# lc700x/desktop2stereo

Measured on AMD Instinct MI355X. Metric: stereo frames/sec @1080p DepthAnything-v2-ViT-B, higher is better.
Workload: dtype bf16; 1 GPU; DepthAnything-v2-vitb bf16, 1920x1080 uint8 RGB noise frames, batch 1 per GPU, Depth Resolution 518 (model input 294x518), Full-SBS uint8 output 3840x1080, pred; parallelism=frame-sharded dp1, no data-path collective (each rank generates its own frames)

## Files before the change

### desktop2stereo_amd/csrc/engine.hip

```cpp
#include <map>
#include <string>
#include <vector>
#include <cmath>
#include <cstring>

#include "gemm.h"
#include "linear_site.h"
#include "vit_ops.h"

using namespace d2s;

namespace {

struct HostT { std::vector<float> data; std::vector<int64_t> shape; };

struct PackedW {
    void* w = nullptr;
    float* bias = nullptr;
    int N = 0, K = 0, Kpad = 0;
};

struct Layer {
    float *ln1g, *ln1b, *ln2g, *ln2b, *ls1, *ls2;
    PackedW qkv, proj, fc1, fc2;
// ... 193 lines not shown
    auto c1 = [&](float x) { return ((A + 2.f) * x - (A + 3.f)) * x * x + 1.f; };
    auto c2 = [&](float x) { return ((A * x - 5.f * A) * x + 8.f * A) * x - 4.f * A; };
    c[0] = c2(t + 1.f); c[1] = c1(t); c[2] = c1(1.f - t); c[3] = c2(2.f - t);
}

void interp_pos(const float* pos, int grid, int D, int gh, int gw, std::vector<float>& out, double offset = 0.0) {
    out.assign((size_t)(1 + gh * gw) * D, 0.f);
    std::memcpy(out.data(), pos, D * sizeof(float));
    if (gh == grid && gw == grid) { std::memcpy(out.data() + D, pos + D, (size_t)grid * grid * D * sizeof(float)); return; }
    float sy = (float)grid / (float)gh, sx = (float)grid / (float)gw;
    if (offset != 0.0) {
        sy = (float)(1.0 / (((double)gh + offset) / (double)grid)); sx = (float)(1.0 / (((double)gw + offset) / (double)grid));
    }
    for (int oy = 0; oy < gh; ++oy) {
        float fy = sy * ((float)oy + 0.5f) - 0.5f;
        float iyf = floorf(fy);
        float cy[4]; cubic_coeffs(fy - iyf, cy);
        int iy = (int)iyf;
        for (int ox = 0; ox < gw; ++ox) {
            float fx = sx * ((float)ox + 0.5f) - 0.5f;
            float ixf = floorf(fx);
            float cx[4]; cubic_coeffs(fx - ixf, cx);
            int ix = (int)ixf;
            float* o = out.data() + (size_t)(1 + oy * gw + ox) * D;
            for (int d = 0; d < D; ++d) {
                float acc = 0.f;
                for (int a = 0; a < 4; ++a) {
                    int yy = std::min(std::max(iy - 1 + a, 0), grid - 1);
                    float row = 0.f;
                    for (int b = 0; b < 4; ++b) {
                        int xx = std::min(std::max(ix - 1 + b, 0), grid - 1);
                        row += pos[(size_t)(1 + yy * grid + xx) * D + d] * cx[b];
                    }
                    acc += row * cy[a];
                }
                o[d] = acc;
            }
        }
    }
}

GemmA plainA(const void* p, long lda) { GemmA a = {}; a.ptr = p; a.mode = A_PLAIN; a.lda = lda; return a; }
GemmA splitA(const void* p, long lda, bool split) { GemmA a = plainA(p, lda); a.bx3 = split ? 1 : 0; return a; }
GemmA convA(const void* p, int Hi, int Wi, int C, int Ho, int Wo, int stride, int relu) {
    GemmA a = {}; a.ptr = p; a.mode = A_CONV3; a.Hi = Hi; a.Wi = Wi; a.C = C; a.Ho = Ho; a.Wo = Wo; a.stride = stride; a.relu = relu; return a;
}

int gemm(d2s_engine* e, const GemmA& a, const PackedW& w, int M, const GemmEpi& ep, hipStream_t st) {
    int Kl = w.K % (e->prec == D2S_PREC_BF16 ? 8 : 4) ? w.Kpad : w.K;
    GemmEpi ep2 = ep;
    if (ep.map == MAP_ROWS) {
        ep2.part = (e->side && st == e->side) ? e->splitk_ws_side : e->splitk_ws;
        ep2.part_elems = e->splitk_elems;
    }
    PROF(a.mode == A_CONV3 ? PC_CONV : PC_GEMM, 2.0 * M * w.N * w.K, 0, launch_gemm(e->wprec, 0, a, w.w, M, w.N, Kl, w.Kpad, ep2, st));
    return D2S_OK;
}

int gemm8(d2s_engine* e, const GemmA& a, const PackedW& w, int M, const GemmEpi& ep, hipStream_t st) {
    PROF(PC_GEMM, 2.0 * M * w.N * w.K, 0, launch_gemm(D2S_PREC_FP8_OPERANDS, 0, a, w.w, M, w.N, w.K, w.Kpad, ep, st));
    return D2S_OK;
}

int conv3(d2s_engine* e, const void* in, int B, int Hi, int Wi, int C, int stride, int relu_in, const PackedW& w,
          void* out, int act, const void* res1, const void* res2, hipStream_t st) {
    int Ho = (Hi + 2 - 3) / stride + 1, Wo = (Wi + 2 - 3) / stride + 1;
    GemmA a = convA(in, Hi, Wi, C, Ho, Wo, stride, relu_in);
    GemmEpi ep = rowsE(out, OUT_T, w.N, w.bias);
    ep.act = act; ep.res1 = res1; ep.res2 = res2;
    return gemm(e, a, w, B * Ho * Wo, ep, st);
}

void window_rows(const d2s_engine::TSlot& sl, bool fold, void* ring, AttnRow& attn, CacheRow& store) {
    const bool in_attn = fold && sl.filled;
    attn = AttnRow{ring, (int16_t)sl.head, (int16_t)(sl.filled ? 32 : 1), in_attn ? sl.head : -1};
    store = CacheRow{ring, sl.filled ? sl.head : 0, sl.filled ? (in_attn ? 0 : 1) : 31};
}

int run_temporal(d2s_engine* e, int m, const void* x, void* out, int B, hipStream_t st, const void* add = nullptr) {
    d2s_engine::TMod& t = e->tm[m];
    const int C = t.C, S = B * t.sites, prec = e->prec;
    const int* ids = e->row_ids;
    const bool fold = e->tm_fold;
    int slots = 0;
    auto producer = [&](GemmEpi& ep) { if (fold) epi_ln_producer(ep, e->tm_a, e->tm_stats, &slots); };
    auto consumer = [&](GemmEpi& ep, const float* csum) { epi_ln_consumer(ep, e->tm_stats, slots, csum, 1e-5f, C); };
    void* gn_out = fold ? e->tm_out : e->tm_a;
    PROF(PC_ELT, 0, 0, launch_groupnorm(prec, x, t.gn_g, t.gn_b, gn_out, t.sites, C, 32, 1e-6f, st, B));
    {
        GemmEpi ep = rowsE(e->tm_hs, OUT_F32, C, t.proj_in.bias);
        producer(ep);
        RC(gemm(e, plainA(gn_out, C), t.proj_in, S, ep, st));
    }
    for (int a = 0; a < 2; ++a) {
        const bool folded = fold && slots >= 1 && slots <= 16;
        if (!folded) PROF(PC_LN, 0, 0, launch_layernorm(prec, e->tm_hs, t.ln_g[a], t.ln_b[a], e->tm_a, S, C, 1e-5f, 0, 0, 0, st));
        {
            GemmEpi ep = rowsE(e->tm_kv, OUT_T, 3 * C, folded ? t.kvq_ln[a].bias : nullptr);
            if (folded) consumer(ep, t.csum_kvq[a]);
            RC(gemm(e, plainA(e->tm_a, C), folded ? t.kvq_ln[a] : t.kvq[a], S, ep, st));
        }
        AttnRows attn = {};
        CacheRows store = {};
        double win_rows = 0;
        bool store_due = false;
        for (int r = 0; r < B; ++r) {
// ... 745 lines not shown
```

### desktop2stereo_amd/csrc/gemm.h

```cpp
#pragma once
#include "common.h"
#include <cstring>

namespace d2s {

enum { A_PLAIN = 0, A_CONV3 = 1 };
enum { ACT_NONE = 0, ACT_GELU = 1, ACT_RELU = 2,
       ACT_GEGLU = 3 };
enum { MAP_ROWS = 0, MAP_SHUFFLE = 1, MAP_QKV = 2, MAP_HEAD = 3 };
enum { OUT_T = 0, OUT_F32 = 1, OUT_BF16 = 2, OUT_BX3 = 3 };

constexpr int D2S_PREC_FP8_OPERANDS = D2S_PREC_FP8;

struct GemmA {
    const void* ptr;
    int mode;
    long lda;
    int Hi, Wi, C;
    int Ho, Wo, stride;
    int relu;
    int buf;
    int bx3;
    int ups, Hs, Ws;
    float usy, usx;
};

constexpr int GEMM_PART_CTR_WORDS = 256;
struct GemmEpi {
    void* out;
    int out_type;
    long ldc;
    const float* bias;
    const float* scale;
    int act;
    const void* res1;
    const void* res2;
    int rows_per_img, img_rows, row_off;
    int res1_mod, res1_off;
    int map, gh, gw, ks, cout;
    void* vt; int ntok, npad, qk_cols, heads;
    float* part; size_t part_elems; int ksplit;
    float head_b3;
    float head_max_depth;
    const float* deq;
    float out_qscale;
    void* out2; float* stats_out; int* stats_slots;
    float out2_qscale;
    int out2_bx3;
    const float* ln_stats; int ln_slots; const float* ln_csum; float ln_eps; int ln_dim;
    int ln_M;
};

int launch_gemm(int precision, int tile, const GemmA& a, const void* W, int M, int N, int K, int Kpad,
                const GemmEpi& e, hipStream_t st);

bool conv3_upsample_ok(int precision, int tile, const GemmA& a, int M, int N, int K, int Kpad, const GemmEpi& e);

int gemm_pp_min_tiles();

enum { GEMM_GLDS = 0, GEMM_HALO = 1, GEMM_CONV3 = 2, GEMM_PP = 3, GEMM_SK = 4 };
enum { NOTE_TAIL_NONE = 0, NOTE_TAIL_INKERNEL = 1, NOTE_TAIL_TWO_LAUNCH = 2, NOTE_TAIL_ROWSPLIT = 3 };
struct GemmPlan {
    int family, inst;
    const char* name;
    int tile;
    unsigned grid, gridy;
    int block;
    unsigned grid2;
    int xn;
    int buf;
    int ksplit, tail;
    int stats_slots;
    int ups;
    int kps, tw, ink, lxn, skew_us;
    const char* error;
};
int plan_gemm(int precision, int tile, const GemmA& a, int M, int N, int K, int Kpad, const GemmEpi& e, GemmPlan& p);

bool plan_conv3_halo2(const GemmA& a, int M, int N, int K, int Kpad, const GemmEpi& e, GemmPlan& p);
void launch_conv3_halo2(const GemmPlan& p, const GemmA& a, const void* W, int M, int N, int Kpad, const GemmEpi& e, hipStream_t st);
bool pp_supported(int precision, const GemmA& a, int M, int N, int K, int Kpad, const GemmEpi& e);
int plan_gemm_pp(int precision, const GemmA& a, int M, int N, int K, int Kpad, const GemmEpi& e, GemmPlan& p);
int launch_gemm_pp(const GemmPlan& p, int precision, const GemmA& a, const void* W, int M, int N, int K, int Kpad, const GemmEpi& e, hipStream_t st);
bool sk_supported(int precision, const GemmA& a, int M, int N, int K, int Kpad, const GemmEpi& e);
void plan_gemm_sk(const GemmA& a, int M, int N, int K, GemmPlan& p);
void launch_gemm_sk(const GemmPlan& p, const GemmA& a, const void* W, int M, int N, int Kpad, const GemmEpi& e, hipStream_t st);

struct KernelNote { const char* name; int tile; int ksplit; int tail; };
KernelNote& kernel_note();

static inline int head_tile(int bn) { return bn == 32 ? 912832 : 9256648; }

static inline size_t conv3_weight_index(int n, int k, int Ci) { const int tap = k / Ci, ci = k % Ci; return ((size_t)n * Ci + ci) * 9 + tap; }

static inline size_t elem_size(int precision) { return precision == D2S_PREC_BF16 ? 2 : (precision == D2S_PREC_FP8_OPERANDS ? 1 : 4); }
static inline void bx3_pack_elem(uint8_t* row, int k, float v) {
    const bf16_t hi = f2bf(v), lo = f2bf(v - bf2f(hi));
    uint8_t* u = row + (size_t)(k >> 3) * 32 + (k & 7) * 2;
    memcpy(u, &hi, 2); memcpy(u + 16, &lo, 2);
}
static inline int gemm_bk(int precision) { return 128 / (int)elem_size(precision); }
static inline int gemm_kpad(int K, int precision) { int bk = 2 * gemm_bk(precision); return (K + bk - 1) / bk * bk; }
static inline int gemm_npad(int N) { return (N + 255) / 256 * 256; }

}
```

### desktop2stereo_amd/csrc/gemm.hip

```cpp
#include "gemm_epi.h"
#include "linear_site.h"
#include <cstdio>
#include <vector>

namespace d2s {

__device__ u32x4 d2s_zero_page[4];

#ifdef D2S_GLDS_TIMING
__device__ unsigned long long glds_timing[4096 * 8];
#define GL_STAMP(SLOT) { if (threadIdx.x == 0 && blockIdx.y == 0 && blockIdx.x < 4096) glds_timing[blockIdx.x * 8 + (SLOT)] = wall_clock64(); }
#else
#define GL_STAMP(SLOT) {}
#endif

typedef short s16x2 __attribute__((ext_vector_type(2)));
typedef short s16x8 __attribute__((ext_vector_type(8)));
__device__ __forceinline__ u32x4 relu_frag(u32x4 v, int floor_bits, bf16_t) {
    s16x8 x = __builtin_bit_cast(s16x8, v);
    short f = (short)floor_bits;
    x = __builtin_elementwise_max(x, (s16x8){f, f, f, f, f, f, f, f});
    return __builtin_bit_cast(u32x4, x);
}
__device__ __forceinline__ u32x4 relu_frag(u32x4 v, int, fp8_t) { return v; }
__device__ __forceinline__ u32x4 relu_frag(u32x4 v, int, bx3_t) { return v; }
__device__ __forceinline__ u32x4 relu_frag(u32x4 v, int floor_bits, float) {
    f32x4 x = __builtin_bit_cast(f32x4, v);
    float f = floor_bits == 0 ? 0.f : -3.0e38f;
    x = __builtin_elementwise_max(x, (f32x4){f, f, f, f});
    return __builtin_bit_cast(u32x4, x);
}

template <int N> __device__ __forceinline__ void wait_vmcnt() { asm volatile("s_waitcnt vmcnt(%0)" ::"n"(N) : "memory"); }

template <int CPR> __device__ __forceinline__ int swz_row(int r) { return CPR == 8 ? ((r >> 1) & 7) : (CPR == 4 ? ((r >> 1) & 3) : (r & 15)); }

static_assert(sizeof(GemmA) + sizeof(GemmEpi) + 8 >= KERNARG_WARM_BYTES, "KERNARG_WARM reads past the kernarg segment");
template <typename T, int BM, int BN, int WM, int WN, int NS, int CPR, int STG = 0>
__global__ void __launch_bounds__(64 * WM * WN)
gemm_glds_kernel(const T* __restrict__ W, const void* a_ptr, long a_lda, int M, int N, int K, int Kpad, int xn, GemmA a, GemmEpi e) {
    static_assert(STG == 0 || STG == 2 || (STG == 1 && NS == 2), "the register-staged variant uses two LDS stages");
    constexpr bool LEAN = STG == 2;
    constexpr bool BX3 = std::is_same<T, bx3_t>::value;
    static_assert(!BX3 || CPR == 8, "bf16x3 units are laid out for 128-byte K tiles");
    constexpr int CE = Prec<T>::CE;
    constexpr int BK = CPR * CE;
    constexpr int RPI = 64 / CPR;
    constexpr int NW = WM * WN;
    constexpr int AI = BM / (RPI * NW), BI = BN / (RPI * NW);
    constexpr int LPT = AI + BI;
    constexpr int FM = BM / WM / 16, FN = BN / WN / 16;
    constexpr int PD = NS - 1;
    constexpr int STAGE = (BM + BN) * CPR;
    __shared__ __attribute__((aligned(16))) u32x4 lds[NS * STAGE];
    KERNARG_WARM(kaw_)
    if constexpr (STG != 2) { KERNARG_WARM_END(kaw_) }
    D2S_POISON_LDS(lds, NS * STAGE)

    const int tid = threadIdx.x, lane = tid & 63;
    const int wid = __builtin_amdgcn_readfirstlane(tid >> 6);
    const int wave_m = wid / WN, wave_n = wid % WN;
    int tm_, tn_;
    GL_STAMP(0)
    if (!tile_of_block(blockIdx.x, (M + BM - 1) / BM, (N + BN - 1) / BN, xn, tm_, tn_)) return;
    const int bm0 = tm_ * BM, bn0 = tn_ * BN;
    static_assert((RPI * NW) % 16 == 0, "row swizzle must be invariant across a thread's instructions");
    static_assert(BM % (RPI * NW) == 0 && BN % (RPI * NW) == 0 && BM % (16 * WM) == 0 && BN % (16 * WN) == 0, "tile must split evenly over the waves");
    const int lrow = wid * RPI + lane / CPR;
    const int src_chunk = (lane % CPR) ^ swz_row<CPR>(lrow);
    const T* zero = (const T*)d2s_zero_page;

    const T* arow[AI];
    int aiy[AI], aix[AI];
    bool aok[AI];
    if constexpr (!LEAN)
#pragma unroll
    for (int i = 0; i < AI; ++i) {
        int m = bm0 + i * NW * RPI + lrow;
        aok[i] = m < M;
        int mm = aok[i] ? m : 0;
        if (a.mode == A_PLAIN) { arow[i] = (const T*)a.ptr + (long)mm * a.lda; aiy[i] = aix[i] = 0; }
        else {
            int ox = mm % a.Wo, oy = (mm / a.Wo) % a.Ho, b = mm / (a.Wo * a.Ho);
            aiy[i] = oy * a.stride - 1; aix[i] = ox * a.stride - 1;
            arow[i] = (const T*)a.ptr + (long)b * a.Hi * a.Wi * a.C;
        }
    }
    const T* wrow = W + (long)(bn0 + lrow) * Kpad + src_chunk * CE;
    const float inv_c = a.mode == A_CONV3 ? 1.0f / (float)a.C : 0.f;
    constexpr int ES = (int)sizeof(T);
    const __amdgpu_buffer_rsrc_t rsA = __builtin_amdgcn_make_buffer_rsrc(uniform_ptr(a_ptr), 0, (unsigned)((long)M * a_lda * ES), 0x00020000);
    const __amdgpu_buffer_rsrc_t rsW = __builtin_amdgcn_make_buffer_rsrc(uniform_ptr(W), 0, (unsigned)((long)((N + 255) / 256 * 256) * Kpad * ES), 0x00020000);
    unsigned voA[AI], voW[BI];
    if constexpr (STG != 1) {
        if (LEAN || a.buf) {
// ... 217 lines not shown
    float2 ln_s[FM];
    float ln_cs[FN][4];
    if (LN_ON && e.ln_csum) {
#pragma unroll
        for (int j = 0; j < FN; ++j) {
            const int n0 = bn0 + wave_n * (BN / WN) + j * 16 + fg * 4;
            if (n0 < N) load4(e.ln_csum + n0, ln_cs[j]);
            else { ln_cs[j][0] = ln_cs[j][1] = ln_cs[j][2] = ln_cs[j][3] = 0.f; }
        }
    }
    constexpr bool PRE = STG == 2 && FM * FN <= 8;
    EpiCols cols[PRE ? FN : 1];
    if constexpr (PRE) {
#pragma unroll
        for (int j = 0; j < FN; ++j) {
            const int n0 = bn0 + wave_n * (BN / WN) + j * 16 + fg * 4;
            if (n0 < N) epi_cols_load(e, n0, cols[j]);
        }
    }
    float pre[PRE ? FM : 1][PRE ? FN : 1][4];
    const bool pre_on = PRE && ksplit == 1 && epi_res1_ahead(e);
    if constexpr (PRE) {
        if (pre_on) {
            static_for<FM>([&](auto ic) {
                constexpr int i = decltype(ic)::value;
                const int m = bm0 + wave_m * (BM / WM) + i * 16 + fr;
                static_for<FN>([&](auto jc) {
                    constexpr int j = decltype(jc)::value;
                    const int n0 = bn0 + wave_n * (BN / WN) + j * 16 + fg * 4;
                    if (m < M && n0 < N) epi_res1_load<T>(e, m, n0, pre[i][j]);
                });
            });
        }
    }
    static_for<FM>([&](auto ic) {
        constexpr int i = decltype(ic)::value;
        const int m = bm0 + wave_m * (BM / WM) + i * 16 + fr;
        float s1 = 0.f, s2 = 0.f;
        float ln_mean = 0.f, ln_rstd = 1.f;
        if (LN_ON && e.ln_csum) {
            float t1 = (lnp[i][0].x + lnp[i][1 % LNS].x) + (lnp[i][2 % LNS].x + lnp[i][3 % LNS].x);
            float t2 = (lnp[i][0].y + lnp[i][1 % LNS].y) + (lnp[i][2 % LNS].y + lnp[i][3 % LNS].y);
            t1 += __shfl_xor(t1, 16); t2 += __shfl_xor(t2, 16);
            t1 += __shfl_xor(t1, 32); t2 += __shfl_xor(t2, 32);
            ln_mean = t1 / (float)e.ln_dim;
            ln_rstd = rsqrtf(fmaxf(t2 / (float)e.ln_dim - ln_mean * ln_mean, 0.f) + e.ln_eps);
        }
        if (m < M) {
            static_for<FN>([&](auto jc) {
                constexpr int j = decltype(jc)::value;
                const int n0 = bn0 + wave_n * (BN / WN) + j * 16 + fg * 4;
                if (n0 < N) {
                    float v[4] = {acc[i][j][0], acc[i][j][1], acc[i][j][2], acc[i][j][3]};
                    if (ksplit > 1) store4(e.part + ((long)blockIdx.y * M + m) * N + n0, v);
                    else {
                        const bool ln = LN_ON && e.ln_csum != nullptr;
                        if (ln) {
                            if (e.deq) { float q[4]; load4(e.deq + n0, q); v[0] *= q[0]; v[1] *= q[1]; v[2] *= q[2]; v[3] *= q[3]; }
                            v[0] = ln_rstd * (v[0] - ln_mean * ln_cs[j][0]); v[1] = ln_rstd * (v[1] - ln_mean * ln_cs[j][1]);
                            v[2] = ln_rstd * (v[2] - ln_mean * ln_cs[j][2]); v[3] = ln_rstd * (v[3] - ln_mean * ln_cs[j][3]);
                        }
                        epilogue_dispatch<T>(e, m, n0, v, ln, PRE && pre_on ? pre[PRE ? i : 0][PRE ? j : 0] : nullptr, PRE ? &cols[PRE ? j : 0] : nullptr);
                        s1 += (v[0] + v[1]) + (v[2] + v[3]);
                        s2 += (v[0] * v[0] + v[1] * v[1]) + (v[2] * v[2] + v[3] * v[3]);
                    }
                }
            });
        }
        if (LN_ON && e.stats_out) {
            s1 += __shfl_xor(s1, 16); s2 += __shfl_xor(s2, 16);
            s1 += __shfl_xor(s1, 32); s2 += __shfl_xor(s2, 32);
            ln_s[i] = make_float2(s1, s2);
        }
    });
    if (LN_ON && e.stats_out) {
        float2* red = (float2*)lds;
        __syncthreads();
#pragma unroll
        for (int i = 0; i < FM; ++i)
            if (fg == 0) red[wave_n * BM + wave_m * (BM / WM) + i * 16 + fr] = ln_s[i];
        __syncthreads();
        for (int r = tid; r < BM; r += 64 * NW) {
            float2 t = red[r];
            for (int w = 1; w < WN; ++w) { t.x += red[w * BM + r].x; t.y += red[w * BM + r].y; }
            if (bm0 + r < M) ((float2*)e.stats_out)[(long)(bn0 / BN) * M + bm0 + r] = t;
        }
    }
#ifdef D2S_GLDS_TIMING
    asm volatile("s_waitcnt vmcnt(0)" ::: "memory");
    GL_STAMP(4)
#endif
}

template <typename T>
__global__ void __launch_bounds__(256)
splitk_reduce_kernel(GemmEpi e, int M, int N) {
    long idx = (long)blockIdx.x * blockDim.x + threadIdx.x;
    int n4 = N >> 2;
    if (idx >= (long)M * n4) return;
    int m = (int)(idx / n4), n0 = (int)(idx % n4) * 4;
    float v[4] = {0.f, 0.f, 0.f, 0.f};
    for (int s = 0; s < e.ksplit; ++s) {
        float p[4];
        load4(e.part + ((long)s * M + m) * N + n0, p);
        v[0] += p[0]; v[1] += p[1]; v[2] += p[2]; v[3] += p[3];
    }
    epilogue_dispatch<T>(e, m, n0, v);
}

template <typename T, int BN, int WM, int WN, int NS = 2>
__global__ void __launch_bounds__(64 * WM * WN)
conv3_halo_kernel(GemmA a, const T* __restrict__ W, int M, int N, int K, int Kpad, GemmEpi e, int xn) {
    KERNARG_WARM(kaw_)
    KERNARG_WARM_END(kaw_)
    constexpr int CE = Prec<T>::CE, CPR = 8, BK = CPR * CE, PD = NS - 1;
    constexpr int TW = 16, TH = 8, BM = TH * TW, HWD = TW + 2, HPX = (TH + 2) * HWD;
    constexpr int HCPP = 16;
    constexpr int NW = WM * WN, RPI = 64 / CPR;
    constexpr int BI = BN / (RPI * NW);
    static_assert(BI >= 1 && BM % (WM * 16) == 0 && BN % (WN * 16) == 0, "bad tile split");
    constexpr int FM = BM / WM / 16, FN = BN / WN / 16;
    constexpr int STAGE = BN * CPR;
    __shared__ __attribute__((aligned(16))) u32x4 lds[NS * STAGE + HPX * HCPP];
    D2S_POISON_LDS(lds, NS * STAGE + HPX * HCPP)
    u32x4* const halo = lds + NS * STAGE;

    const int tid = threadIdx.x, lane = tid & 63;
// ... 152 lines not shown
};

static constexpr int glds_codes[][2] = {{256128, G_256128}, {128, G_128}, {64, G_64}, {3264, G_3264}, {1281288, G_1281288},
                                        {641288, G_641288}, {64648, G_64648}, {256648, G_256648}, {128324, G_128324}, {964, G_964},
                                        {91288, G_91288}, {912832, G_912832}, {9256648, G_9256648}};
static constexpr struct { int code, alias, auto_of, inst; } bx3_codes[] = {
    {93264, 3264, 3264, G_93264}, {964, 64, 64648, G_964}, {964128, 0, 641288, G_964128}, {91288, 128, 1281288, G_91288},
    {912832, 0, 912832, G_912832}, {9256648, 0, 9256648, G_9256648}};

#define HALO_INSTANCES(X) X(H_64, 64,4,2,4) X(H_128, 128,2,4,2)
enum {
#define X(ID, ...) ID,
    HALO_INSTANCES(X)
#undef X
};
static constexpr struct { int BN, WM, WN, NS; } halo_cfg[] = {
#define X(ID, ...) {__VA_ARGS__},
    HALO_INSTANCES(X)
#undef X
};
static const char* const halo_names[][4] = {
#define X(ID, ...) {"conv3_halo_kernel<bf16," #__VA_ARGS__ ">", nullptr, "conv3_halo_kernel<f32," #__VA_ARGS__ ">", nullptr},
    HALO_INSTANCES(X)
#undef X
};

static inline int type_index(int precision) {
    return precision == D2S_PREC_BF16 ? 0 : (precision == D2S_PREC_FP8_OPERANDS ? 1 : (precision == D2S_PREC_BF16X3 ? 3 : 2));
}
template <typename T> constexpr int type_bit() {
    return std::is_same<T, bf16_t>::value ? TY_BF16 : std::is_same<T, fp8_t>::value ? TY_E4M3 : std::is_same<T, bx3_t>::value ? TY_BX3 : TY_F32;
}

static int plan_fail(GemmPlan& p, int rc, const char* msg) { p.error = msg; return rc; }
static int glds_inst_of(int code) {
    for (const auto& c : glds_codes) if (c[0] == code) return c[1];
    return -1;
}

static int plan_glds(int inst, int precision, int tile, const GemmA& a, int M, int N, int K, int Kpad, const GemmEpi& e, GemmPlan& p) {
    const GldsCfg& c = glds_cfg[inst];
    const int es = (int)elem_size(precision), bk = c.CPR * (16 / es);
    p.family = GEMM_GLDS; p.inst = inst; p.name = glds_names[inst][type_index(precision)]; p.tile = tile; p.block = 64 * c.WM * c.WN;
    p.xn = pick_xn(cdiv(M, c.BM), cdiv(N, c.BN), c.BN, Kpad, es, p.grid);
    const int nkt = cdiv(K, bk);
    int ks = 1;
    if (c.STG != 2 && e.part && e.part_elems > 0 && !e.stats_out && (int)p.grid < SPLITK_GRID && nkt >= 24) {
        ks = nkt / 6; if (ks > 16) ks = 16;
        while (ks > 1 && (size_t)ks * M * N > e.part_elems) --ks;
    }
    static EnvInt sk_force{"D2S_SPLITK_FORCE", 0};
    if (sk_force.get() > 1 && c.STG != 2 && e.part && !e.stats_out && nkt >= sk_force.get() && (size_t)sk_force.get() * M * N <= e.part_elems) ks = sk_force.get();
    p.ksplit = ks; p.gridy = ks;
    if (ks > 1) { p.grid2 = cdiv((long)M * (N / 4), 256); return D2S_OK; }
    p.stats_slots = c.WN > 1 ? cdiv(N, c.BN) : 1 << 20;
    p.buf = c.STG != 1 && buf_eligible(a, M, N, K, Kpad, bk, es);
    return D2S_OK;
}

static int lean_of(int t, int precision, const GemmA& a, int M, int N, int K, int Kpad, const GemmEpi& e) {
    const int inst = t == 3264 ? G_L3264 : (t == 64648 ? G_L64648 : (t == 641288 ? G_L641288 : -1));
    if (inst < 0 || !gemm_deep() || !buf_eligible(a, M, N, K, Kpad, gemm_bk(precision), elem_size(precision))) return -1;
    const long tiles = (long)cdiv(M, glds_cfg[inst].BM) * cdiv(N, glds_cfg[inst].BN);
    return tiles <= 512 && !splitk_wanted(e, tiles, K, gemm_bk(precision)) ? inst : -1;
}

static int small_tile_of(int M, int N) {
    const long b128 = (long)cdiv(M, 128) * cdiv(N, 128), b64128 = (long)cdiv(M, 64) * cdiv(N, 128), b64 = (long)cdiv(M, 64) * cdiv(N, 64);
    if (b128 >= 400 && (N >= 1536 || b128 >= 900)) return 1281288;
    if (b64128 >= 280) return 641288;
    if (b64 >= 384) return 64648;
    return 3264;
}

static int auto_tile(int M, int N) {
    if (N <= 64) return (long)cdiv(M, 256) >= 224 ? (N <= 32 ? 912832 : 9256648) : 3264;
    return small_tile_of(M, N);
}

static bool plan_halo(int precision, const GemmA& a, int M, int N, int K, int Kpad, const GemmEpi& e, GemmPlan& p) {
    static EnvInt off{"D2S_NO_HALO", 0};
    if (off.get() || precision == D2S_PREC_FP8_OPERANDS) return false;
    const int es = (int)elem_size(precision), cpp = a.C * es / 16;
    if (a.mode != A_CONV3 || a.stride != 1 || a.Hi != a.Ho || a.Wi != a.Wo || (a.C * es) % 128 || cpp > 16 || (cpp & (cpp - 1))) return false;
    if (e.map != MAP_ROWS || e.rows_per_img || K != 9 * a.C || N <= 32) return false;
    const int nimg = M / (a.Ho * a.Wo);
    const long tiles_m = (long)nimg * cdiv(a.Ho, 8) * cdiv(a.Wo, 16);
    if (tiles_m * cdiv(N, 128) < 200 || (long)nimg * a.Ho * a.Wo != M) return false;
    const int inst = N <= 64 ? H_64 : H_128, bn = halo_cfg[inst].BN;
    p.family = GEMM_HALO; p.inst = inst; p.block = 64 * halo_cfg[inst].WM * halo_cfg[inst].WN; p.ups = a.ups;
    p.name = halo_names[inst][type_index(precision)];
    p.xn = pick_xn((int)tiles_m, cdiv(N, bn), bn, Kpad, es, p.grid);
    return true;
}

int gemm_pp_min_tiles() {
    static EnvInt v{"D2S_GEMM_PP", 100};
    return v.get();
}

int plan_gemm(int precision, int tile, const GemmA& a, int M, int N, int K, int Kpad, const GemmEpi& e, GemmPlan& p) {
    p = GemmPlan{};
    p.gridy = 1; p.ksplit = 1; p.buf = a.buf; p.stats_slots = -1;
    const int ce = 16 / (int)elem_size(precision);
    if (M <= 0 || N <= 0 || K <= 0 || (N & 3) || (K % ce) || Kpad % (2 * gemm_bk(precision)))
        return plan_fail(p, D2S_E_INVALID, "launch_gemm: bad dims (N % 4, K % chunk, Kpad % BK)");
    if (a.mode == A_PLAIN && (a.lda % ce)) return plan_fail(p, D2S_E_INVALID, "launch_gemm: lda not chunk aligned");
    if (a.mode == A_CONV3 && (a.C % ce)) return plan_fail(p, D2S_E_INVALID, "launch_gemm: conv channels not chunk aligned");
    if (precision == D2S_PREC_BF16X3) {
        if (e.deq || (e.out2 && !e.out2_bx3))
            return plan_fail(p, D2S_E_UNSUPPORTED, "launch_gemm: bf16x3 operands: no de-quantisation, raw-residual copies in the unit format only");
        if (a.bx3) {
            if (a.mode != A_PLAIN || a.relu) return plan_fail(p, D2S_E_UNSUPPORTED, "launch_gemm: a pre-split bf16x3 A operand must be a plain matrix");
            const int t = small_tile_of(M, N), lean = lean_of(t, precision, a, M, N, K, Kpad, e);
            return plan_glds(lean >= 0 ? lean : glds_inst_of(t), precision, t, a, M, N, K, Kpad, e, p);
        }
        if (tile == 256256) tile = 0;
        const int t = tile ? tile : auto_tile(M, N);
        for (const auto& c : bx3_codes)
            if (tile ? (tile == c.code || tile == c.alias) : t == c.auto_of) return plan_glds(c.inst, precision, tile ? tile : c.code, a, M, N, K, Kpad, e, p);
        return plan_fail(p, D2S_E_INVALID, "launch_gemm: bad tile code for bf16x3 operands");
    }
    if (tile == 256256) return plan_gemm_pp(precision, a, M, N, K, Kpad, e, p);
    if (precision == D2S_PREC_BF16 && a.mode == A_CONV3 && (tile == 0 || e.map == MAP_HEAD) && plan_conv3_halo2(a, M, N, K, Kpad, e, p)) return D2S_OK;
    if (a.ups) {
        if (precision == D2S_PREC_BF16 && tile == 0 && plan_halo(precision, a, M, N, K, Kpad, e, p)) return D2S_OK;
        return plan_fail(p, D2S_E_UNSUPPORTED, "launch_gemm: this launch cannot fold the up-sample into its loader (conv3_upsample_ok says when)");
    }
    if (precision == D2S_PREC_FP8_OPERANDS && (a.mode != A_PLAIN || a.relu)) return plan_fail(p, D2S_E_UNSUPPORTED, "launch_gemm: e4m3 operands are for plain linears");
    if (tile == 0 && plan_halo(precision, a, M, N, K, Kpad, e, p)) return D2S_OK;
    if (tile == 0 && sk_supported(precision, a, M, N, K, Kpad, e)) { plan_gemm_sk(a, M, N, K, p); return D2S_OK; }
    const int pp_min_tiles = gemm_pp_min_tiles();
    if (tile == 0 && pp_min_tiles > 0 && (long)cdiv(M, 256) * cdiv(N, 256) >= pp_min_tiles && pp_supported(precision, a, M, N, K, Kpad, e))
        return plan_gemm_pp(precision, a, M, N, K, Kpad, e, p);
    if (tile == 0) {
        tile = auto_tile(M, N);
        if (N > 64 && a.mode == A_CONV3 && K >= 4096 && (long)cdiv(M, 128) * cdiv(N, 128) >= 300) tile = 1281288;
    }
    if ((precision == D2S_PREC_BF16 || precision == D2S_PREC_FP8_OPERANDS) && !(e.part && e.ksplit > 1) && e.map != MAP_HEAD) {
        const int lean = lean_of(tile, precision, a, M, N, K, Kpad, e);
        if (lean >= 0) return plan_glds(lean, precision, tile, a, M, N, K, Kpad, e, p);
    }
    const int inst = glds_inst_of(tile);
    if (inst < 0) return plan_fail(p, D2S_E_INVALID, "launch_gemm: bad tile code");
    return plan_glds(inst, precision, tile, a, M, N, K, Kpad, e, p);
}

bool conv3_upsample_ok(int precision, int tile, const GemmA& a, int M, int N, int K, int Kpad, const GemmEpi& e) {
    static EnvInt no_ups{"D2S_NO_UPSFOLD", 0};
    if (no_ups.get() || precision != D2S_PREC_BF16 || a.mode != A_CONV3 || !a.ups || a.Hs < 2 || a.Ws < 2 || a.usy <= 0.f || a.usx <= 0.f) return false;
    GemmPlan p;
    return plan_gemm(precision, tile, a, M, N, K, Kpad, e, p) == D2S_OK && p.ups;
}

template <typename T>
static void launch_glds(const GemmPlan& p, const GemmA& a, const void* W, int M, int N, int K, int Kpad, const GemmEpi& e, hipStream_t st) {
    const dim3 grid(p.grid, p.gridy), block(p.block);
    if (p.family == GEMM_HALO) {
        if constexpr ((type_bit<T>() & (TY_BF16 | TY_F32)) != 0) switch (p.inst) {
#define X(ID, ...) case ID: hipLaunchKernelGGL((conv3_halo_kernel<T, __VA_ARGS__>), grid, block, 0, st, a, (const T*)W, M, N, K, Kpad, e, p.xn); break;
            HALO_INSTANCES(X)
#undef X
        }
        return;
    }
    switch (p.inst) {
#define X(ID, TY, ...) case ID: if constexpr (((TY) & type_bit<T>()) != 0) \
        hipLaunchKernelGGL((gemm_glds_kernel<T, __VA_ARGS__>), grid, block, 0, st, (const T*)W, a.ptr, a.lda, M, N, K, Kpad, p.xn, a, e); break;
        GLDS_INSTANCES(X)
#undef X
    }
    if (p.grid2) hipLaunchKernelGGL((splitk_reduce_kernel<T>), dim3(p.grid2), dim3(256), 0, st, e, M, N);
}

static void note_kernel(const GemmPlan& p) { kernel_note() = KernelNote{p.name, p.tile, p.ksplit, p.tail}; }

int launch_gemm(int precision, int tile, const GemmA& a, const void* W, int M, int N, int K, int Kpad,
                const GemmEpi& e, hipStream_t st) {
    GemmPlan p;
    if (const int rc = plan_gemm(precision, tile, a, M, N, K, Kpad, e, p)) { set_error(p.error); return rc; }
    note_kernel(p);
    if (e.stats_slots && p.stats_slots >= 0) *e.stats_slots = p.stats_slots;
    GemmA a1 = a;
    a1.buf = p.buf;
    GemmEpi e1 = e;
    e1.ksplit = p.family == GEMM_GLDS ? p.ksplit : 1;
    switch (p.family) {
        case GEMM_CONV3: launch_conv3_halo2(p, a1, W, M, N, Kpad, e1, st); break;
        case GEMM_SK: launch_gemm_sk(p, a1, W, M, N, Kpad, e1, st); break;
        case GEMM_PP: if (const int rc = launch_gemm_pp(p, precision, a1, W, M, N, K, Kpad, e1, st)) return rc; break;
        default:
            if (precision == D2S_PREC_BF16) launch_glds<bf16_t>(p, a1, W, M, N, K, Kpad, e1, st);
            else if (precision == D2S_PREC_FP8_OPERANDS) launch_glds<fp8_t>(p, a1, W, M, N, K, Kpad, e1, st);
            else if (precision == D2S_PREC_BF16X3) launch_glds<bx3_t>(p, a1, W, M, N, K, Kpad, e1, st);
            else launch_glds<float>(p, a1, W, M, N, K, Kpad, e1, st);
    }
    D2S_CHECK_LAUNCH();
    return D2S_OK;
}

__global__ void cast_pad_kernel(const float* __restrict__ src, void* __restrict__ dst, int rows, int cols,
                                int rows_pad, int cols_pad, int prec) {
    long idx = (long)blockIdx.x * blockDim.x + threadIdx.x;
    if (idx >= (long)rows_pad * cols_pad) return;
    int c = (int)(idx % cols_pad), r = (int)(idx / cols_pad);
    float v = (r < rows && c < cols) ? src[(long)r * cols + c] : 0.f;
    if (prec == -D2S_PREC_BF16X3) {
        const bf16_t hi = f2bf(v), lo = f2bf(v - bf2f(hi));
        bf16_t* u = (bf16_t*)((char*)dst + ((long)r * cols_pad + (c & ~7)) * 4) + (c & 7);
        u[0] = hi; u[8] = lo;
    } else
    if (prec == D2S_PREC_BF16) ((bf16_t*)dst)[idx] = f2bf(v);
    else if (prec == D2S_PREC_FP8_OPERANDS) ((fp8_t*)dst)[idx] = f2e4m3(v);
    else ((float*)dst)[idx] = v;
}

}

using namespace d2s;

namespace d2s {

static thread_local KernelNote g_kernel_note = {};
KernelNote& kernel_note() { return g_kernel_note; }

namespace {
struct ProbeBuf {
    void* p = nullptr;
    ProbeBuf() = default;
    ProbeBuf(const ProbeBuf&) = delete;
    ProbeBuf& operator=(const ProbeBuf&) = delete;
    ~ProbeBuf() { if (p) (void)hipFree(p); }
};

int fetch_f32(std::vector<float>& h, const float* d, size_t n) {
    h.resize(n);
    D2S_HIP(hipMemcpy(h.data(), d, n * sizeof(float), hipMemcpyDeviceToHost));
    return D2S_OK;
}
int upload(ProbeBuf& buf, const void* h, size_t bytes) {
    D2S_HIP(hipMalloc(&buf.p, bytes));
    D2S_HIP(hipMemcpy(buf.p, h, bytes, hipMemcpyHostToDevice));
    return D2S_OK;
}

int alloc_splitk_ws(ProbeBuf& buf, size_t elems, hipStream_t st) {
    const size_t bytes = (elems + GEMM_PART_CTR_WORDS) * sizeof(float);
    D2S_HIP(hipMalloc(&buf.p, bytes));
    D2S_HIP(hipMemsetAsync(buf.p, 0, bytes, st));
    return D2S_OK;
}

std::string noted_kernel() {
    const KernelNote kn = kernel_note();
    std::string name = kn.name ? kn.name : "unrecorded";
    if (kn.name && !strncmp(kn.name, "gemm_glds_kernel", 16)) {
        name += " tile=" + std::to_string(kn.tile);
        if (kn.ksplit > 1) name += " splitk=" + std::to_string(kn.ksplit);
    } else if (kn.name && kn.tail != NOTE_TAIL_NONE) {
        static const char* const tails[4] = {"", "in-kernel", "two-launch", "row-split"};
        name += " ks=" + std::to_string(kn.ksplit) + " tail=" + tails[kn.tail];
    }
    return name;
}
}

}

extern "C" int d2s_gemm_probe(const float* A, const float* Wt, const float* bias, float* Cout, int M, int N, int K,
                              int precision, int tile, int iters, void* stream) {
    D2S_REQUIRE(A && Wt && Cout && M > 0 && N > 0 && K > 0 && (N % 4 == 0) && iters >= 1, "bad argument");
    D2S_REQUIRE(precision == D2S_PREC_BF16 || precision == D2S_PREC_FP32 || precision == D2S_PREC_FP8_OPERANDS || precision == D2S_PREC_BF16X3, "bad precision");
    hipStream_t st = (hipStream_t)stream;
    int bf = precision;
    int Kp = gemm_kpad(K, precision), Np = gemm_npad(N);
    size_t es = elem_size(precision);
    ProbeBuf dA, dW, dP;
    D2S_HIP(hipMalloc(&dA.p, (size_t)M * Kp * es));
    D2S_HIP(hipMalloc(&dW.p, (size_t)Np * Kp * es));
    hipLaunchKernelGGL(cast_pad_kernel, dim3(cdiv((long)M * Kp, 256)), dim3(256), 0, st, A, dA.p, M, K, M, Kp, bf);
    hipLaunchKernelGGL(cast_pad_kernel, dim3(cdiv((long)Np * Kp, 256)), dim3(256), 0, st, Wt, dW.p, N, K, Np, Kp, bf == D2S_PREC_BF16X3 ? -bf : bf);
    GemmA a = {};
    a.ptr = dA.p; a.mode = A_PLAIN; a.lda = Kp;
    GemmEpi e = {};
    e.out = Cout; e.out_type = OUT_F32; e.ldc = N; e.bias = bias;
    static EnvInt sk_force{"D2S_SPLITK_FORCE", 0};
    if (sk_force.get() > 1) {
        const size_t pe = (size_t)sk_force.get() * M * N;
        int rc = alloc_splitk_ws(dP, pe, st);
        if (rc != D2S_OK) return rc;
        e.part = (float*)dP.p; e.part_elems = pe;
    }
    int rc = D2S_OK;
    for (int i = 0; i < iters && rc == D2S_OK; ++i) rc = launch_gemm(precision, tile, a, dW.p, M, N, Kp, Kp, e, st);
    hipError_t err = hipStreamSynchronize(st);
    if (rc != D2S_OK) return rc;
    D2S_HIP(err);
    return D2S_OK;
}

extern "C" int d2s_conv3_probe(d2s_conv3_probe_params* p, void* stream) {
    D2S_REQUIRE(p && p->struct_size == sizeof(d2s_conv3_probe_params), "d2s_conv3_probe_params.struct_size must be sizeof(d2s_conv3_probe_params)");
    p->kernel[0] = 0;
    const int prec = p->precision, B = p->batch, C = p->C, N = p->N;
    D2S_REQUIRE(prec == D2S_PREC_BF16 || prec == D2S_PREC_FP32 || prec == D2S_PREC_BF16X3, "bad precision (bf16, fp32 or bf16x3)");
    D2S_REQUIRE(p->x && p->w && p->out && B > 0 && C > 0 && N > 0 && p->Hs > 0 && p->Ws > 0 && p->Hi > 0 && p->Wi > 0, "bad argument");
    D2S_REQUIRE(p->stride == 1 || p->stride == 2, "stride must be 1 or 2");
    const bool ups = p->Hs != p->Hi || p->Ws != p->Wi;
    D2S_REQUIRE(!ups || p->stride == 1, "a folded up-sample needs stride 1");
    D2S_REQUIRE(!p->map_head || (p->w3 && !p->res && p->act == 0 && p->stride == 1), "map_head: w3 needed; no residual, no act, stride 1");
    hipStream_t st = (hipStream_t)stream;
    const int Ho = (p->Hi + 2 - 3) / p->stride + 1, Wo = (p->Wi + 2 - 3) / p->stride + 1;
    const long M = (long)B * Ho * Wo, nsrc = (long)B * p->Hs * p->Ws;
    D2S_REQUIRE(M < (1L << 31) && nsrc * C < (1L << 31), "too large");
    const int K = 9 * C, Kp = gemm_kpad(K, prec);
    const bool bf = prec == D2S_PREC_BF16;
    const bool out_t = !p->out_f32 && !p->map_head;
    ProbeBuf dW, dX, dR, dP;
    {
        std::vector<float> w;
        int rc = fetch_f32(w, p->w, (size_t)N * C * 9);
        if (rc == D2S_OK) {
            const LinearImage im = prepare_linear(prec, N, K, [&](int n, int k) { return w[conv3_weight_index(n, k, C)]; }, nullptr);
            rc = upload(dW, im.w.data(), im.w.size());
        }
        if (rc != D2S_OK) return rc;
    }
    const void* x = p->x;
    if (bf) {
        D2S_HIP(hipMalloc(&dX.p, (size_t)nsrc * C * 2));
        hipLaunchKernelGGL(cast_pad_kernel, dim3(cdiv(nsrc * C, 256)), dim3(256), 0, st, p->x, dX.p, (int)nsrc, C, (int)nsrc, C, D2S_PREC_BF16);
        x = dX.p;
    }
    const void* res = p->res;
    if (res && bf && out_t) {
        D2S_HIP(hipMalloc(&dR.p, (size_t)M * N * 2));
        hipLaunchKernelGGL(cast_pad_kernel, dim3(cdiv(M * N, 256)), dim3(256), 0, st, p->res, dR.p, (int)M, N, (int)M, N, D2S_PREC_BF16);
        res = dR.p;
    }
    D2S_HIP(hipExtGetLastError());
    GemmA a = {};
    a.ptr = x; a.mode = A_CONV3; a.Hi = p->Hi; a.Wi = p->Wi; a.C = C; a.Ho = Ho; a.Wo = Wo; a.stride = p->stride; a.relu = p->relu_in;
    if (ups) { a.ups = 1; a.Hs = p->Hs; a.Ws = p->Ws; a.usy = linear_scale(p->Hs, p->Hi, true); a.usx = linear_scale(p->Ws, p->Wi, true); }
    GemmEpi e = {};
    e.out = p->out; e.out_type = out_t ? OUT_T : OUT_F32; e.ldc = N; e.bias = p->bias;
    e.act = p->act ? ACT_RELU : ACT_NONE; e.res1 = res;
    if (p->map_head) { e.ldc = 1; e.map = MAP_HEAD; e.scale = p->w3; e.head_b3 = p->b3; e.head_max_depth = p->max_depth; }
    const int tile = p->tile ? p->tile : (p->map_head ? head_tile(N <= 32 ? 32 : 64) : 0);
    if (p->splitk_elems > 0) {
        int rc = alloc_splitk_ws(dP, (size_t)p->splitk_elems, st);
        if (rc != D2S_OK) return rc;
        e.part = (float*)dP.p; e.part_elems = (size_t)p->splitk_elems;
    }
    if (ups && !conv3_upsample_ok(prec, tile, a, (int)M, N, K, Kp, e)) {
        set_error("d2s_conv3_probe: conv3_upsample_ok refuses to fold this up-sample");
        return D2S_E_UNSUPPORTED;
    }
    kernel_note() = KernelNote{nullptr, 0, 1};
    int rc = launch_gemm(prec, tile, a, dW.p, (int)M, N, K, Kp, e, st);
    hipError_t err = hipStreamSynchronize(st);
    if (rc != D2S_OK) return rc;
    D2S_HIP(err);
    snprintf(p->kernel, sizeof(p->kernel), "%s", noted_kernel().c_str());
    return D2S_OK;
}

namespace d2s {
namespace {
enum { ACT_F32 = 0, ACT_BF16 = 1, ACT_BX3 = 2, ACT_E4M3 = 3 };
size_t act_bytes(int fmt) { return fmt == ACT_BF16 ? 2 : (fmt == ACT_E4M3 ? 1 : 4); }

int act_operand(ProbeBuf& buf, const float* x, int M, int K, int lda, int fmt, float qscale) {
    std::vector<float> h;
    int rc = fetch_f32(h, x, (size_t)M * K);
    if (rc != D2S_OK) return rc;
    std::vector<uint8_t> o((size_t)M * lda * act_bytes(fmt), 0);
    for (int m = 0; m < M; ++m)
        for (int k = 0; k < K; ++k) {
            const float v = h[(size_t)m * K + k];
            const size_t i = (size_t)m * lda + k;
            if (fmt == ACT_BF16) ((bf16_t*)o.data())[i] = f2bf(v);
            else if (fmt == ACT_E4M3) o[i] = f2e4m3(v * qscale);
            else if (fmt == ACT_BX3) bx3_pack_elem(o.data() + (size_t)m * lda * 4, k, v);
            else ((float*)o.data())[i] = v;
        }
    return upload(buf, o.data(), o.size());
}

struct ProbeLinear {
    ProbeBuf w, bias, csum, deq;
    int Kp = 0;
};
int upload_linear(ProbeLinear& L, const LinearImage& im, float s_a) {
    L.Kp = im.Kpad;
    int rc = upload(L.w, im.w.data(), im.w.size());
    if (rc == D2S_OK && !im.bias.empty()) rc = upload(L.bias, im.bias.data(), im.bias.size() * sizeof(float));
    if (rc == D2S_OK && !im.csum.empty()) rc = upload(L.csum, im.csum.data(), im.csum.size() * sizeof(float));
    if (rc == D2S_OK && !im.sw.empty()) {
        const std::vector<float> dq = deq_scales(s_a, im.sw);
        rc = upload(L.deq, dq.data(), dq.size() * sizeof(float));
    }
    return rc;
}
}
}

extern "C" int d2s_linear_probe(d2s_linear_probe_params* p, void* stream) {
    D2S_REQUIRE(p && p->struct_size == sizeof(d2s_linear_probe_params), "d2s_linear_probe_params.struct_size must be sizeof(d2s_linear_probe_params)");
    p->kernel[0] = 0; p->kernel2[0] = 0; p->stats_slots = 0;
    const int prec = p->precision, site = p->site, M = p->M, N = p->N, K = p->K;
    D2S_REQUIRE(prec == D2S_PREC_FP32 || prec == D2S_PREC_BF16 || prec == D2S_PREC_BF16X3 || prec == D2S_PREC_FP8 || prec == D2S_PREC_FP8_MLP, "bad precision");
    D2S_REQUIRE(site >= D2S_LIN_PATCH && site <= D2S_LIN_TM_PROJ_OUT, "bad site");
    D2S_REQUIRE(M > 0 && N > 0 && K > 0 && p->w, "bad argument");
    hipStream_t st = (hipStream_t)stream;
    const PrecRules pr = prec_rules(prec);
    const int wprec = pr.w, aprec = pr.act;
    const bool x3 = wprec == D2S_PREC_BF16X3, f8 = pr.e4m3;
    const bool enc = site == D2S_LIN_QKV || site == D2S_LIN_PROJ || site == D2S_LIN_FC1 || site == D2S_LIN_FC2;
    const bool e8 = pr.e4m3_site(site);
    const bool fold = p->ln_fold != 0;
    const bool consumer = fold && (site == D2S_LIN_QKV || site == D2S_LIN_FC1 || site == D2S_LIN_NECK_PROJ || site == D2S_LIN_TM_KVQ || site == D2S_LIN_TM_FF1);
    const bool producer = fold && !consumer;
    D2S_REQUIRE(!producer || site == D2S_LIN_PROJ || site == D2S_LIN_FC2 || site == D2S_LIN_TM_PROJ_IN || site == D2S_LIN_TM_TO_OUT || site == D2S_LIN_TM_FF2,
                "ln_fold: not a LayerNorm consumer or producer site");
    D2S_REQUIRE(!fold || (pr.ln_folds(site) && (enc || !f8)), "ln_fold: the engine does not fold LayerNorm there in this precision");
    const bool per_frame = site == D2S_LIN_QKV || site == D2S_LIN_PATCH || site == D2S_LIN_NECK_PROJ;
    const int P = p->ntok - 1;
    D2S_REQUIRE(!per_frame || (p->ntok > 1 && M % (site == D2S_LIN_PATCH ? P : p->ntok) == 0), "M must be a multiple of the rows per frame");
    const int B = per_frame ? M / (site == D2S_LIN_PATCH ? P : p->ntok) : 1;
    D2S_REQUIRE(site != D2S_LIN_QKV || (p->vt && p->heads > 0 && N == 3 * K && K == 64 * p->heads && p->npad >= p->ntok), "QKV: N = 3 K, K = 64 heads, vt, npad >= ntok");
    D2S_REQUIRE(site != D2S_LIN_NECK_RESIZE || (p->ks > 0 && p->gh > 0 && p->gw > 0 && N == p->ks * p->ks * K && M % (p->gh * p->gw) == 0), "NECK_RESIZE: N = ks^2 K, M = B gh gw");
    D2S_REQUIRE(site != D2S_LIN_TM_FF1 || !consumer || N % 8 == 0, "GEGLU: N must be a multiple of 8");
    D2S_REQUIRE(!x3 || (site != D2S_LIN_QKV && site != D2S_LIN_FC1) || (N % 8 == 0 && K % 8 == 0), "bf16x3 unit-format outputs: whole units (N % 8 == 0)");
    D2S_REQUIRE(!consumer || (p->pa && p->pw && p->pK > 0 && p->ln_g && p->ln_b && p->x && p->out2 && p->stats), "ln_fold consumer: pa, pw, ln_g, ln_b, x, out2, stats");
    D2S_REQUIRE(!producer || (p->out2 && (site == D2S_LIN_TM_FF2 || p->stats)), "ln_fold producer: out2, stats");
    const bool x_out = site == D2S_LIN_PATCH || site == D2S_LIN_PROJ || site == D2S_LIN_FC2 || site == D2S_LIN_TM_PROJ_IN || site == D2S_LIN_TM_TO_OUT || site == D2S_LIN_TM_FF2;
    D2S_REQUIRE(x_out ? p->x != nullptr : p->out != nullptr, "x (residual-stream sites) / out needed");
    ProbeBuf ws;
    if (p->splitk_elems > 0) { int rc = alloc_splitk_ws(ws, (size_t)p->splitk_elems, st); if (rc != D2S_OK) return rc; }
    auto launch = [&](bool fp8_ops, const GemmA& a, const ProbeLinear& L, int rows, int n, int Kl, GemmEpi ep, char* name) -> int {
        if (!fp8_ops && ep.map == MAP_ROWS && ws.p) { ep.part = (float*)ws.p; ep.part_elems = (size_t)p->splitk_elems; }
        kernel_note() = KernelNote{nullptr, 0, 1, NOTE_TAIL_NONE};
        int rc = launch_gemm(fp8_ops ? D2S_PREC_FP8_OPERANDS : wprec, p->tile, a, L.w.p, rows, n, Kl, L.Kp, ep, st);
        if (rc != D2S_OK) return rc;
        snprintf(name, 128, "%s", noted_kernel().c_str());
        return D2S_OK;
    };
    auto ragged_k = [&](int k, int kp) { return k % (aprec == D2S_PREC_BF16 ? 8 : 4) ? kp : k; };
    const int ofmt = x3 ? ACT_BX3 : ((consumer ? e8 : f8) ? ACT_E4M3 : ACT_BF16);
    const float o2q = ofmt == ACT_E4M3 ? 1.0f / p->s_res : 0.f;
    int slots = 0;
    ProbeBuf dPa;
    ProbeLinear Lp;
    if (consumer) {
        const bool p8 = pr.e4m3_attn;
        const int pK = p->pK, D = K;
        std::vector<float> hw, hb;
        int rc = fetch_f32(hw, p->pw, (size_t)D * pK);
        if (rc == D2S_OK && p->pbias) rc = fetch_f32(hb, p->pbias, D);
        if (rc != D2S_OK) return rc;
        rc = upload_linear(Lp, prepare_linear(p8 ? D2S_PREC_FP8_OPERANDS : wprec, D, pK, [&](int n, int k) { return hw[(size_t)n * pK + k]; },
                                              p->pbias ? hb.data() : nullptr), p->s_pact);
        if (rc != D2S_OK) return rc;
        const int pfmt = p8 ? ACT_E4M3 : (x3 ? ACT_BX3 : (aprec == D2S_PREC_BF16 ? ACT_BF16 : ACT_F32));
        rc = act_operand(dPa, p->pa, M, pK, pK, pfmt, p8 ? 1.0f / p->s_pact : 0.f);
        if (rc != D2S_OK) return rc;
        GemmA a = {}; a.ptr = dPa.p; a.mode = A_PLAIN; a.lda = pK; a.bx3 = pfmt == ACT_BX3;
        GemmEpi ep = epi_residual(p->x, D, (const float*)Lp.bias.p, p->pscale);
        epi_ln_producer(ep, p->out2, p->stats, &slots, x3, o2q);
        if (p8) ep.deq = (const float*)Lp.deq.p;
        rc = launch(p8, a, Lp, M, D, p8 ? pK : ragged_k(pK, Lp.Kp), ep, p->kernel2);
        if (rc != D2S_OK) return rc;
        p->stats_slots = slots;
        if (slots < 1 || slots > 16) { set_error("d2s_linear_probe: the producer leaves no statistics a consumer takes (the engine runs the LayerNorm kernel)"); return D2S_E_UNSUPPORTED; }
    }
    ProbeLinear L;
    {
        std::vector<float> hw, hb, hg, hbt, pb;
        const int Co = site == D2S_LIN_NECK_RESIZE ? K : 0, ks = p->ks;
        int rc = fetch_f32(hw, p->w, (size_t)N * K);
        if (rc == D2S_OK && p->bias) rc = fetch_f32(hb, p->bias, Co ? Co : N);
        if (rc == D2S_OK && consumer) rc = fetch_f32(hg, p->ln_g, K);
        if (rc == D2S_OK && consumer) rc = fetch_f32(hbt, p->ln_b, K);
        if (rc != D2S_OK) return rc;
        const bool geglu = consumer && site == D2S_LIN_TM_FF1;
        auto row = [&](int n) { return geglu ? geglu_row(n, N / 8) : n; };
        auto at = [&](int n, int k) { return Co ? hw[convT_weight_index(n, k, Co, ks)] : hw[(size_t)row(n) * K + k]; };
        if (p->bias) { pb.resize(N); for (int n = 0; n < N; ++n) pb[n] = Co ? hb[n % Co] : hb[row(n)]; }
        rc = upload_linear(L, prepare_linear(e8 ? D2S_PREC_FP8_OPERANDS : wprec, N, K, at, p->bias ? pb.data() : nullptr, consumer ? hg.data() : nullptr,
                                             consumer ? hbt.data() : nullptr), consumer ? p->s_res : p->s_act);
        if (rc != D2S_OK) return rc;
    }
    ProbeBuf dA, dR, dR2;
    const int afmt = consumer ? ofmt : (e8 ? ACT_E4M3 : (x3 && enc ? ACT_BX3 : (aprec == D2S_PREC_BF16 ? ACT_BF16 : ACT_F32)));
// ... 61 lines not shown
```

Baseline: 889.1 stereo frames/s.

## Fuse split-K reduction into the 32x64 GEMM via last-arriving tile counter

For bf16 split-K GEMMs using the 32x64 glds tile, each split writes its partials with cache-bypassing stores and bumps a per-tile atomic counter. The last-arriving block sums all slabs and runs the epilogue itself, so the separate reduction kernel launch is skipped. This trades a launch and an extra pass for atomics, coherence-bypassing loads and serialized tail work in one block per tile. It is gated by an environment mask that is on by default and by a limit on the number of tile counters.

```diff
diff --git a/desktop2stereo_amd/csrc/engine.hip b/desktop2stereo_amd/csrc/engine.hip
--- a/desktop2stereo_amd/csrc/engine.hip
+++ b/desktop2stereo_amd/csrc/engine.hip
@@ -269,6 +269,7 @@
     if (ep.map == MAP_ROWS) {
         ep2.part = (e->side && st == e->side) ? e->splitk_ws_side : e->splitk_ws;
         ep2.part_elems = e->splitk_elems;
+        ep2.ink = e->prec == D2S_PREC_BF16 && tail_fuse(TAIL_FUSE_SPLITK);
     }
     PROF(a.mode == A_CONV3 ? PC_CONV : PC_GEMM, 2.0 * M * w.N * w.K, 0, launch_gemm(e->wprec, 0, a, w.w, M, w.N, Kl, w.Kpad, ep2, st));
     return D2S_OK;
diff --git a/desktop2stereo_amd/csrc/gemm.h b/desktop2stereo_amd/csrc/gemm.h
--- a/desktop2stereo_amd/csrc/gemm.h
+++ b/desktop2stereo_amd/csrc/gemm.h
@@ -39,7 +39,7 @@
     int res1_mod, res1_off;
     int map, gh, gw, ks, cout;
     void* vt; int ntok, npad, qk_cols, heads;
-    float* part; size_t part_elems; int ksplit;
+    float* part; size_t part_elems; int ksplit; int ink;
     float head_b3;
     float head_max_depth;
     const float* deq;
@@ -57,6 +57,9 @@
 bool conv3_upsample_ok(int precision, int tile, const GemmA& a, int M, int N, int K, int Kpad, const GemmEpi& e);
 
 int gemm_pp_min_tiles();
+
+enum { TAIL_FUSE_SPLITK = 1 };
+bool tail_fuse(int bit);
 
 enum { GEMM_GLDS = 0, GEMM_HALO = 1, GEMM_CONV3 = 2, GEMM_PP = 3, GEMM_SK = 4 };
 enum { NOTE_TAIL_NONE = 0, NOTE_TAIL_INKERNEL = 1, NOTE_TAIL_TWO_LAUNCH = 2, NOTE_TAIL_ROWSPLIT = 3 };
diff --git a/desktop2stereo_amd/csrc/gemm.hip b/desktop2stereo_amd/csrc/gemm.hip
--- a/desktop2stereo_amd/csrc/gemm.hip
+++ b/desktop2stereo_amd/csrc/gemm.hip
@@ -33,6 +33,16 @@
 
 template <int N> __device__ __forceinline__ void wait_vmcnt() { asm volatile("s_waitcnt vmcnt(%0)" ::"n"(N) : "memory"); }
 
+__device__ __forceinline__ void store4_through(float* p, const float v[4]) {
+    const f32x4 x = {v[0], v[1], v[2], v[3]};
+    asm volatile("global_store_dwordx4 %0, %1, off sc0 sc1" ::"v"(p), "v"(x) : "memory");
+}
+__device__ __forceinline__ f32x4 load4_sc1(const float* base , unsigned byte_off) {
+    f32x4 v;
+    asm volatile("global_load_dwordx4 %0, %1, %2 sc1" : "=&v"(v) : "v"(byte_off), "s"(base) : "memory");
+    return v;
+}
+
 template <int CPR> __device__ __forceinline__ int swz_row(int r) { return CPR == 8 ? ((r >> 1) & 7) : (CPR == 4 ? ((r >> 1) & 3) : (r & 15)); }
 
 static_assert(sizeof(GemmA) + sizeof(GemmEpi) + 8 >= KERNARG_WARM_BYTES, "KERNARG_WARM reads past the kernarg segment");
@@ -41,6 +51,7 @@
 gemm_glds_kernel(const T* __restrict__ W, const void* a_ptr, long a_lda, int M, int N, int K, int Kpad, int xn, GemmA a, GemmEpi e) {
     static_assert(STG == 0 || STG == 2 || (STG == 1 && NS == 2), "the register-staged variant uses two LDS stages");
     constexpr bool LEAN = STG == 2;
+    constexpr bool INK = STG == 0 && BM == 32 && BN == 64;
     constexpr bool BX3 = std::is_same<T, bx3_t>::value;
     static_assert(!BX3 || CPR == 8, "bf16x3 units are laid out for 128-byte K tiles");
     constexpr int CE = Prec<T>::CE;
@@ -364,8 +375,10 @@
                 const int n0 = bn0 + wave_n * (BN / WN) + j * 16 + fg * 4;
                 if (n0 < N) {
                     float v[4] = {acc[i][j][0], acc[i][j][1], acc[i][j][2], acc[i][j][3]};
-                    if (ksplit > 1) store4(e.part + ((long)blockIdx.y * M + m) * N + n0, v);
-                    else {
+                    if (ksplit > 1) {
+                        float* dst = e.part + ((long)blockIdx.y * M + m) * N + n0;
+                        if (INK && e.ink) store4_through(dst, v); else store4(dst, v);
+                    } else {
                         const bool ln = LN_ON && e.ln_csum != nullptr;
                         if (ln) {
                             if (e.deq) { float q[4]; load4(e.deq + n0, q); v[0] *= q[0]; v[1] *= q[1]; v[2] *= q[2]; v[3] *= q[3]; }
@@ -385,6 +398,45 @@
             ln_s[i] = make_float2(s1, s2);
         }
     });
+    if constexpr (INK) {
+        if (ksplit > 1 && e.ink) {
+            asm volatile("s_waitcnt vmcnt(0)" ::: "memory");
+            __syncthreads();
+            volatile unsigned* sh = (volatile unsigned*)lds;
+            unsigned* ctr = (unsigned*)(e.part + e.part_elems) + tm_ * ((N + BN - 1) / BN) + tn_;
+            if (tid == 0) sh[0] = __hip_atomic_fetch_add(ctr, 1u, __ATOMIC_RELAXED, __HIP_MEMORY_SCOPE_AGENT);
+            __syncthreads();
+            if (sh[0] != (unsigned)ksplit - 1) return;
+            if (tid == 0) __hip_atomic_store(ctr, 0u, __ATOMIC_RELAXED, __HIP_MEMORY_SCOPE_AGENT);
+            constexpr int RQ = 16;
+            const long slab = (long)M * N;
+            const int m = bm0 + wave_m * (BM / WM) + fr, n0 = bn0 + wave_n * (BN / WN) + fg * 4;
+            const bool ok0 = m < M && n0 < N, ok1 = m < M && n0 + 16 < N;
+            const unsigned vo0 = ok0 ? (unsigned)(((long)m * N + n0) * 4) : 0u, vo1 = ok1 ? vo0 + 64u : 0u;
+            float v0[4] = {0.f, 0.f, 0.f, 0.f}, v1[4] = {0.f, 0.f, 0.f, 0.f};
+            for (int s0 = 0; s0 < ksplit; s0 += RQ) {
+                f32x4 x0[RQ], x1[RQ];
+#pragma unroll
+                for (int q = 0; q < RQ; ++q)
+                    if (s0 + q < ksplit) {
+                        const float* range = (const float*)uniform_ptr(e.part + (s0 + q) * slab);
+                        x0[q] = load4_sc1(range, vo0);
+                        x1[q] = load4_sc1(range, vo1);
+                    }
+                asm volatile("s_waitcnt vmcnt(0)" ::: "memory");
+#pragma unroll
+                for (int q = 0; q < RQ; ++q)
+                    if (s0 + q < ksplit) {
+                        asm volatile("" : "+v"(x0[q]), "+v"(x1[q]));
+                        v0[0] += x0[q][0]; v0[1] += x0[q][1]; v0[2] += x0[q][2]; v0[3] += x0[q][3];
+                        v1[0] += x1[q][0]; v1[1] += x1[q][1]; v1[2] += x1[q][2]; v1[3] += x1[q][3];
+                    }
+            }
+            if (ok0) epilogue_dispatch<T>(e, m, n0, v0);
+            if (ok1) epilogue_dispatch<T>(e, m, n0 + 16, v1);
+            return;
+        }
+    }
     if (LN_ON && e.stats_out) {
         float2* red = (float2*)lds;
         __syncthreads();
@@ -643,7 +695,11 @@
     static EnvInt sk_force{"D2S_SPLITK_FORCE", 0};
     if (sk_force.get() > 1 && c.STG != 2 && e.part && !e.stats_out && nkt >= sk_force.get() && (size_t)sk_force.get() * M * N <= e.part_elems) ks = sk_force.get();
     p.ksplit = ks; p.gridy = ks;
-    if (ks > 1) { p.grid2 = cdiv((long)M * (N / 4), 256); return D2S_OK; }
+    if (ks > 1) {
+        p.ink = e.ink && inst == G_3264 && (long)cdiv(M, c.BM) * cdiv(N, c.BN) <= GEMM_PART_CTR_WORDS;
+        if (!p.ink) p.grid2 = cdiv((long)M * (N / 4), 256);
+        return D2S_OK;
+    }
     p.stats_slots = c.WN > 1 ? cdiv(N, c.BN) : 1 << 20;
     p.buf = c.STG != 1 && buf_eligible(a, M, N, K, Kpad, bk, es);
     return D2S_OK;
@@ -688,6 +744,11 @@
 int gemm_pp_min_tiles() {
     static EnvInt v{"D2S_GEMM_PP", 100};
     return v.get();
+}
+
+bool tail_fuse(int bit) {
+    static EnvInt mask{"D2S_TAIL_FUSE", TAIL_FUSE_SPLITK};
+    return (mask.get() & bit) != 0;
 }
 
 int plan_gemm(int precision, int tile, const GemmA& a, int M, int N, int K, int Kpad, const GemmEpi& e, GemmPlan& p) {
@@ -776,6 +837,7 @@
     a1.buf = p.buf;
     GemmEpi e1 = e;
     e1.ksplit = p.family == GEMM_GLDS ? p.ksplit : 1;
+    e1.ink = p.family == GEMM_GLDS && p.ksplit > 1 ? p.ink : 0;
     switch (p.family) {
         case GEMM_CONV3: launch_conv3_halo2(p, a1, W, M, N, Kpad, e1, st); break;
         case GEMM_SK: launch_gemm_sk(p, a1, W, M, N, Kpad, e1, st); break;
@@ -881,6 +943,7 @@
         int rc = alloc_splitk_ws(dP, pe, st);
         if (rc != D2S_OK) return rc;
         e.part = (float*)dP.p; e.part_elems = pe;
+        e.ink = precision == D2S_PREC_BF16 && tail_fuse(TAIL_FUSE_SPLITK);
     }
     int rc = D2S_OK;
     for (int i = 0; i < iters && rc == D2S_OK; ++i) rc = launch_gemm(precision, tile, a, dW.p, M, N, Kp, Kp, e, st);
@@ -942,8 +1005,9 @@
         int rc = alloc_splitk_ws(dP, (size_t)p->splitk_elems, st);
         if (rc != D2S_OK) return rc;
         e.part = (float*)dP.p; e.part_elems = (size_t)p->splitk_elems;
-    }
-    if (ups && !conv3_upsample_ok(prec, tile, a, (int)M, N, K, Kp, e)) {
+        e.ink = bf && tail_fuse(TAIL_FUSE_SPLITK);
+    }
+    if (ups &&!conv3_upsample_ok(prec, tile, a, (int)M, N, K, Kp, e)) {
         set_error("d2s_conv3_probe: conv3_upsample_ok refuses to fold this up-sample");
         return D2S_E_UNSUPPORTED;
     }
@@ -1030,7 +1094,10 @@
     ProbeBuf ws;
     if (p->splitk_elems > 0) { int rc = alloc_splitk_ws(ws, (size_t)p->splitk_elems, st); if (rc != D2S_OK) return rc; }
     auto launch = [&](bool fp8_ops, const GemmA& a, const ProbeLinear& L, int rows, int n, int Kl, GemmEpi ep, char* name) -> int {
-        if (!fp8_ops && ep.map == MAP_ROWS && ws.p) { ep.part = (float*)ws.p; ep.part_elems = (size_t)p->splitk_elems; }
+        if (!fp8_ops && ep.map == MAP_ROWS && ws.p) {
+            ep.part = (float*)ws.p; ep.part_elems = (size_t)p->splitk_elems;
+            ep.ink = prec == D2S_PREC_BF16 && tail_fuse(TAIL_FUSE_SPLITK);
+        }
         kernel_note() = KernelNote{nullptr, 0, 1, NOTE_TAIL_NONE};
         int rc = launch_gemm(fp8_ops ? D2S_PREC_FP8_OPERANDS : wprec, p->tile, a, L.w.p, rows, n, Kl, L.Kp, ep, st);
         if (rc != D2S_OK) return rc;
```

Result: slower. 877.4 stereo frames/s (-1.3%).
